# akhilmurthy/spacedrive

Measured on AMD Instinct MI355X. Metric: cas_id files/sec + BLAKE3 GB/s hashed (node) at 1/2/4/8 MI355X, higher is better.
Workload: dtype u32

## Files before the change

### spacedrive_amd/csrc/b3_batch.h

```cpp
#pragma once
#include <hip/hip_runtime.h>
#include <stddef.h>
#include <stdint.h>

namespace sdcas {

constexpr uint32_t kTile = 1024;
constexpr uint32_t kWG = 512;
constexpr uint32_t kSmallTile = 128;
constexpr uint64_t kSmallSlots = 1ull << 14;
constexpr int kSmallVariant = 84;
constexpr uint32_t kSortTotalsWords = 256;
constexpr uint32_t kSortPerWG = 4096;
inline size_t sort_key_words(size_t max_msgs) { return kSortTotalsWords + 256 * (max_msgs / kSortPerWG + 1); }

struct BatchWorkspace {
  uint64_t* S = nullptr;
  uint32_t* tile_first = nullptr;
  uint64_t* total = nullptr;
  uint32_t* nodes = nullptr;
  void* scan_tmp = nullptr;
  size_t scan_tmp_bytes = 0;
  uint32_t cap_msgs = 0;
  uint64_t cap_chunks = 0;
  uint64_t cap_slots = 0;
  int variant = -1;
  uint64_t small_slots = kSmallSlots;
  int small_variant = kSmallVariant;
  uint64_t cap_small_tiles = 0;
  int sort = 1;
  uint32_t* perm = nullptr;
  uint64_t* soffs = nullptr;
  uint64_t* slens = nullptr;
  uint32_t* sort_keys = nullptr;
};

size_t batch_scan_temp_bytes(uint32_t max_msgs);
int leaf_variant();
int leaf_variant_count();
bool leaf_variant_available(int v);
bool leaf_variant_forced();
bool piece_variant_available(int v);

constexpr uint32_t kSortMinMsgs = 128;
struct BatchPlan {
  const uint64_t* S = nullptr;
  const uint32_t* tile_first = nullptr;
  uint64_t* total = nullptr;
  uint32_t tile = 0;
  bool crossing = true;
};
uint64_t batch_plan_host(const uint64_t* lens, uint32_t n, uint32_t tile, uint64_t cap_slots, uint64_t* S,
                         uint32_t* tile_first, uint64_t* total, bool* crossing);

hipError_t batch_hash(const BatchWorkspace& ws, const uint8_t* blob, const uint64_t* offs, const uint64_t* lens,
                      uint32_t n, uint8_t* out32, uint64_t* out_keys, hipStream_t st, uint64_t max_chunks = 0,
                      hipEvent_t ev0 = nullptr, hipEvent_t ev1 = nullptr, const BatchPlan* plan = nullptr);

hipError_t plan_slots(const uint64_t* lens, uint32_t n, void* tmp, size_t tmp_bytes, uint64_t cap_slots, uint64_t* S,
                      uint32_t* tile_first, uint64_t* total, hipStream_t st);
hipError_t finish_crossing(uint64_t tiles, const uint64_t* lens, uint32_t n, const uint64_t* S,
                           const uint32_t* tile_first, const uint64_t* total, uint64_t cap_slots,
                           const uint32_t* nodes, uint8_t* out32, uint64_t* out_keys, hipStream_t st);

constexpr uint64_t kWholeMax = 102400;
constexpr uint64_t kGatherStride = 57360;
constexpr uint32_t kIdentifyMaxSampled = 4096;
struct IdentifyScratch {
  uint8_t* p = nullptr;
  size_t bytes = 0;
};
size_t identify_scratch_bytes(uint32_t n, uint32_t sampled_cap);
hipError_t identify_hash(const BatchWorkspace& ws, const IdentifyScratch& sc, const uint8_t* blob,
                         const uint64_t* offs, const uint64_t* lens, uint32_t n, uint32_t sampled_cap,
                         uint64_t* out_keys, uint8_t* out32, uint8_t* out_has_key, hipStream_t st);

struct PieceDesc {
  uint64_t off;
  uint64_t j0;
  uint64_t node_base;
  uint32_t len;
  uint32_t pad;
};
struct SegDesc {
  uint64_t off;
  uint64_t j0;
  uint64_t node_base;
  uint64_t len;
  uint64_t piece_first;
};
struct FileDesc {
  uint64_t C;
  uint64_t node_base;
  uint64_t out_index;
};
inline uint64_t bigfile_node_count(uint64_t C) {
  return C / kTile + (uint64_t)__builtin_popcountll(C % kTile);
// ... 11 lines not shown
```

### spacedrive_amd/csrc/b3_batch.hip

```cpp
#include <hip/hip_runtime.h>

#include <atomic>
#ifdef SDCAS_ABLATIONS
#include <hipcub/hipcub.hpp>
#endif
#include <stdint.h>
#include <cstdio>
#include <cstring>

#include "b3_device.h"
#include "b3_batch.h"
#include "b3_tree.h"

namespace sdcas {

using namespace b3d;

constexpr int kMaxStack = 64;
constexpr int kMaxStackBig = 64;


template <uint32_t TILE = kTile>
__global__ void k_tile_first(const uint64_t* __restrict__ lens, const uint64_t* __restrict__ S, uint32_t n,
                             uint64_t cap_chunks, uint32_t* __restrict__ tile_first, uint64_t* __restrict__ total) {
// ... 372 lines not shown
    static_assert(L == 8 || L == 9 || L == 4 || L == 59 || L == 69 || L == 79 || L == 89, "ablation block loops need -DSDCAS_ABLATIONS");
#endif
  }
}

template <int PF>
__device__ __forceinline__ const uint8_t* leaf_ptr(const uint8_t* blob, const uint8_t* p) {
#ifdef SDCAS_ABLATIONS
  return leaf_ptr_ablation<PF>(blob, p);
#else
  (void)blob;
  return p;
#endif
}

__device__ __forceinline__ uint32_t leaf_bin(uint64_t len, uint64_t j) {
  const uint64_t rest = len - j * CHUNK_LEN;
  const uint32_t clen = len == 0 ? 0u : (uint32_t)min<uint64_t>(CHUNK_LEN, rest);
  const uint32_t nb = clen == 0 ? 1u : (clen + BLOCK_LEN - 1) / BLOCK_LEN;
  return 16u - nb;
}


template <int WG, uint32_t NB = 17, uint32_t TL = kTile>
__device__ __forceinline__ void leaf_order(uint32_t tid, const uint32_t (&bin)[TL / WG], uint16_t* __restrict__ order,
                                           uint16_t* __restrict__ gcnt) {
  constexpr uint32_t kGroups = TL / 64;
  const uint32_t lane = tid & 63;
  uint32_t rk[TL / WG];
#pragma unroll
  for (uint32_t r = 0; r < TL / WG; ++r) {
    const uint32_t g = (tid + r * WG) >> 6;
    uint32_t mine = 0, cnt_l = 0;
#pragma unroll 1
    for (uint32_t b = 0; b < NB; ++b) {
      const uint64_t m = __ballot(bin[r] == b);
      if (bin[r] == b) mine = __builtin_amdgcn_mbcnt_hi((uint32_t)(m >> 32), __builtin_amdgcn_mbcnt_lo((uint32_t)m, 0u));
      if (lane == b) cnt_l = (uint32_t)__popcll(m);
    }
    rk[r] = mine;
    if (lane < NB) gcnt[lane * kGroups + g] = (uint16_t)cnt_l;
  }
  __syncthreads();
  if (tid < 64) {
    constexpr uint32_t kPer = (NB * kGroups + 63) / 64;
    uint32_t v[kPer], sum = 0;
#pragma unroll
    for (uint32_t q = 0; q < kPer; ++q) {
      const uint32_t e = tid * kPer + q;
      v[q] = e < NB * kGroups ? gcnt[e] : 0u;
      sum += v[q];
    }
    uint32_t inc = sum;
#pragma unroll
    for (uint32_t d = 1; d < 64; d <<= 1) {
      const uint32_t t = __shfl_up(inc, d);
      if (lane >= d) inc += t;
    }
    uint32_t acc = inc - sum;
#pragma unroll
    for (uint32_t q = 0; q < kPer; ++q) {
      const uint32_t e = tid * kPer + q;
      if (e < NB * kGroups) gcnt[e] = (uint16_t)acc;
      acc += v[q];
    }
  }
  __syncthreads();
#pragma unroll
  for (uint32_t r = 0; r < TL / WG; ++r) {
    const uint32_t s = tid + r * WG;
    order[gcnt[bin[r] * kGroups + (s >> 6)] + rk[r]] = (uint16_t)s;
  }
  __syncthreads();
}

template <int WG, int PF, int TR = 1, int ORD = 0, int DYN = 0, int CA = 0, int MINW = 0, uint32_t TL = kTile,
          int QD = 0, int XT = 0>
__global__ void __launch_bounds__(WG, MINW ? MINW : (ORD ? 6 : 1)) k_leaf_tree(const uint8_t* __restrict__ blob, const uint64_t* __restrict__ offs,
                                                   const uint64_t* __restrict__ lens, uint32_t n,
                                                   const uint64_t* __restrict__ S,
                                                   const uint32_t* __restrict__ tile_first,
                                                   const uint64_t* __restrict__ total_p, uint64_t cap_chunks,
                                                   uint32_t* __restrict__ nodes, uint8_t* __restrict__ out32,
                                                   uint64_t* __restrict__ out_keys, const uint32_t* __restrict__ perm) {
  __shared__ uint32_t cvs[TL][8];
  __shared__ uint64_t sS[TL + 1];
  __shared__ uint16_t smsg[TL];
  __shared__ uint32_t task[kTaskCap<TL>];
  __shared__ uint32_t ntask[12];
  __shared__ uint16_t order[ORD ? TL : 1];
  __shared__ uint32_t sexp[(XT & 2) ? TL / 32 : 1];
  __shared__ uint64_t next_tile;
  __shared__ uint32_t qbuf[QD == 3 ? 16 * (WG / 4) : 1];

  if constexpr (((XT >> 3) & 7) != 0) asm volatile(".rept %c0\n s_nop 0\n .endr" ::"i"((XT >> 3) & 7));
  const uint64_t total = *total_p;
  if (total > cap_chunks) return;
  const uint64_t ntiles = (total + TL - 1) / TL;
  const uint32_t tid = threadIdx.x;
  static_assert(!QD || (ORD == 0 && CA == 0 && WG % 4 == 0), "quad slots: no leaf order, no cached chunk");
  constexpr uint32_t SW = QD ? WG / 4 : WG;
  const uint32_t sid = QD ? tid >> 2 : tid;
  const bool lead = !QD || (tid & 3u) == 0;
  const uint32_t qslot = 16 * sid;
  uint32_t wi[QD == 3 ? 28 : 1];
  if constexpr (QD == 3) {
    const uint32_t q = tid & 3u;
    const bool q1 = q & 1u, q2 = q & 2u;
#pragma unroll
    for (int k = 0; k < 28; ++k)
      wi[k] = qslot + qsel(q1, q2, kQuadWord.w[0][k], kQuadWord.w[1][k], kQuadWord.w[2][k], kQuadWord.w[3][k]);
  }
  unsigned long long* tile_ctr = reinterpret_cast<unsigned long long*>(const_cast<uint64_t*>(total_p) + 2);
  for (uint64_t tile = blockIdx.x; tile < ntiles;) {
    const uint64_t tbase = tile * TL;
    const uint32_t m0 = tile_first[tile];
    const uint32_t m1 = (tile + 1 < ntiles) ? tile_first[tile + 1] : n - 1;
    const uint32_t cnt = m1 - m0 + 1;
    for (uint32_t i = tid; i < cnt; i += WG) sS[i] = S[m0 + i];
    if (tid < 12) ntask[tid] = 0;
    if constexpr ((XT & 2) != 0)
      for (uint32_t i = tid; i < TL / 32; i += WG) sexp[i] = 0;
    if (DYN == 1 && tid == 0) next_tile = gridDim.x + atomicAdd(tile_ctr, 1ull);
    __syncthreads();

    constexpr uint32_t R = TL / SW;
    const uint8_t* c_p[R];
    uint64_t c_j[R];
    uint32_t c_clen[R], c_m[R];
    bool c_ok[R], c_root[R];
#pragma unroll
    for (uint32_t r = 0; r < R; ++r) c_ok[r] = false;
    constexpr uint32_t kPhase1Unroll = CA ? R : 1;
#pragma unroll kPhase1Unroll
    for (uint32_t s = sid; s < TL; s += SW) {
      const uint64_t g = tbase + s;
      uint32_t K = 0;
      if (g >= total) {
        smsg[s] = kNoMsg;
      } else {
        uint32_t lo = 0, hi = cnt - 1;
        while (lo < hi) {
          const uint32_t mid = (lo + hi + 1) >> 1;
          if (sS[mid] <= g) lo = mid;
          else hi = mid - 1;
        }
        smsg[s] = (uint16_t)lo;
        if (TR || CA) {
          const uint64_t j = g - sS[lo];
          const uint64_t len = lens[m0 + lo];
          const uint64_t C = chunk_count(len);
          if (CA && (CA == 1 || s == tid)) {
            const uint32_t r = (s - tid) / WG;
            c_ok[r] = true;
            c_m[r] = m0 + lo;
            c_j[r] = j;
            c_clen[r] = len == 0 ? 0u : (uint32_t)min<uint64_t>(CHUNK_LEN, len - j * CHUNK_LEN);
            c_root[r] = C == 1;
            c_p[r] = blob + offs[m0 + lo] + j * CHUNK_LEN;
          }
          if (TR && C != 1 && lead) {
            K = node_level_t<TL>(j, C, s);
            if constexpr ((XT & 4) == 0)
              for (uint32_t k = 1; k <= K; ++k)
                task[task_base<TL>(k) + atomicAdd(&ntask[k], 1u)] = enc_task(s, s + (1u << (k - 1)), 0, false);
            if constexpr ((XT & 2) != 0) {
              const uint64_t S0 = g - j;
              if ((S0 < tbase || S0 + C > tbase + TL) && !parent_in_tile_t<TL>(j, C, s, K))
                atomicOr(&sexp[s >> 5], 1u << (s & 31));
            }
          }
        }
      }
      if constexpr ((XT & 4) != 0) {
        for (uint32_t k = 1;; ++k) {
          const bool want = K >= k;
          const uint64_t bal = __ballot(want);
          if (!bal) break;
          const uint32_t first = (uint32_t)__ffsll((long long)bal) - 1;
          uint32_t base = 0;
          if (__lane_id() == first) base = atomicAdd(&ntask[k], (uint32_t)__popcll(bal));
          base = __shfl(base, (int)first);
          const uint32_t below =
              __builtin_amdgcn_mbcnt_hi((uint32_t)(bal >> 32), __builtin_amdgcn_mbcnt_lo((uint32_t)bal, 0u));
          if (want) task[task_base<TL>(k) + base + below] = enc_task(s, s + (1u << (k - 1)), 0, false);
        }
      }
    }
#pragma unroll 1
    for (uint32_t i = sid; TR && lead && i < cnt; i += SW) {
      const uint64_t S0 = sS[i];
      if (S0 < tbase) continue;
      const uint64_t C = chunk_count(lens[m0 + i]);
      if (C == 1 || S0 + C > tbase + TL) continue;
      const uint32_t s0 = (uint32_t)(S0 - tbase), c = (uint32_t)C;
      if (!(c & (c - 1))) {
        const uint32_t k = 31 - __clz(c);
// ... 218 lines not shown
template <uint32_t TILE, bool QUAD = false, class At>
__device__ __forceinline__ void merge_nodes_flat(const uint32_t* __restrict__ nodes, uint64_t s0, uint64_t C, At at,
                                                 uint32_t (&cv)[8]) {
  int depth = 0, keep = 0;
  uint64_t j = 0;
  uint32_t k = 0;
  bool have = false, done = false;
  uint32_t v[8];
  for (;;) {
    int op = 0;
    while (!done) {
      if (!have) {
        const uint64_t g = s0 + j;
        k = node_level_t<TILE>(j, C, (uint32_t)(g % TILE));
        const uint4* p = reinterpret_cast<const uint4*>(nodes + 8ull * g);
        const uint4 a = p[0], b = p[1];
        v[0] = a.x; v[1] = a.y; v[2] = a.z; v[3] = a.w;
        v[4] = b.x; v[5] = b.y; v[6] = b.z; v[7] = b.w;
        keep = __popcll(j);
        have = true;
      }
      if (depth > keep) {
        op = 1;
        break;
      }
      if (j + (1ull << k) < C) {
        uint32_t* pp = at(depth);
#pragma unroll
        for (int i = 0; i < 8; ++i) pp[i] = v[i];
        ++depth;
        j += 1ull << k;
        have = false;
        continue;
      }
      if (depth == 0) {
#pragma unroll
        for (int i = 0; i < 8; ++i) cv[i] = v[i];
        done = true;
        break;
      }
      op = 2;
      break;
    }
    if (__builtin_amdgcn_ballot_w64(op != 0) == 0) return;
    if (op) {
      uint32_t l[8], r[8], o[8];
      const uint32_t* pl = at(op == 1 ? depth - 2 : depth - 1);
      const uint32_t* pr = at(depth - 1);
#pragma unroll
      for (int i = 0; i < 8; ++i) {
        l[i] = pl[i];
        r[i] = op == 1 ? pr[i] : v[i];
      }
      if constexpr (QUAD) parent_quad(l, r, op == 2 && depth == 1, o);
      else parent(l, r, op == 2 && depth == 1, o);
      if (op == 1) {
        uint32_t* po = at(depth - 2);
#pragma unroll
        for (int i = 0; i < 8; ++i) po[i] = o[i];
      } else {
#pragma unroll
        for (int i = 0; i < 8; ++i) v[i] = o[i];
      }
      --depth;
    }
  }
}

template <uint32_t TILE>
__device__ __noinline__ void merge_nodes_deep(const uint32_t* __restrict__ nodes, uint64_t s0, uint64_t C,
                                              uint32_t (&cv)[8]) {
  uint32_t stack[kMaxStack][8];
  merge_nodes<TILE>(nodes, s0, C, [&](int d) { return &stack[d][0]; }, cv);
}

constexpr int kFinishWG = 64, kFinishDepth = 24;
template <uint32_t TILE>
__global__ void __launch_bounds__(kFinishWG) k_finish_t(const uint64_t* __restrict__ lens, uint32_t n,
                                                       const uint64_t* __restrict__ S,
                                                       const uint32_t* __restrict__ tile_first,
                                                       const uint64_t* __restrict__ total_p, uint64_t cap_slots,
                                                       const uint32_t* __restrict__ nodes,
                                                       const uint32_t* __restrict__ perm, uint8_t* __restrict__ out32,
                                                       uint64_t* __restrict__ out_keys) {
  constexpr uint32_t kFinishRow = kFinishDepth * 8 + 1;
  __shared__ uint32_t lstack[kFinishWG][kFinishRow];
  const uint64_t t = (uint64_t)blockIdx.x * blockDim.x + threadIdx.x;
  const uint64_t total = *total_p;
  if (total > cap_slots || t == 0 || t * TILE >= total) return;
  const uint32_t m = tile_first[t];
  const uint64_t s0 = S[m];
  if (s0 >= t * TILE || s0 / TILE != t - 1) return;
  const uint64_t C = chunk_count(lens[m]);
  if (s0 + C <= t * TILE) return;
  uint32_t cv[8];
  if (C < (1ull << (kFinishDepth - 2)))
    merge_nodes_flat<TILE>(nodes, s0, C, [&](int d) { return &lstack[threadIdx.x][8 * d]; }, cv);
  else
    merge_nodes_deep<TILE>(nodes, s0, C, cv);
  store_digest(perm ? perm[m] : m, cv, out32, out_keys);
}

constexpr int kFinishQWG = 64, kFinishQPerWG = kFinishQWG / 4;
template <uint32_t TILE>
__global__ void __launch_bounds__(kFinishQWG) k_finish_q(const uint64_t* __restrict__ lens, uint32_t n,
                                                        const uint64_t* __restrict__ S,
                                                        const uint32_t* __restrict__ tile_first,
                                                        const uint64_t* __restrict__ total_p, uint64_t cap_slots,
                                                        const uint32_t* __restrict__ nodes,
                                                        const uint32_t* __restrict__ perm, uint8_t* __restrict__ out32,
                                                        uint64_t* __restrict__ out_keys) {
  constexpr uint32_t kFinishRow = kFinishDepth * 8 + 1;
  __shared__ uint32_t lstack[kFinishQPerWG][kFinishRow];
  const uint32_t b = threadIdx.x >> 2;
  const uint64_t t = (uint64_t)blockIdx.x * kFinishQPerWG + b;
  const uint64_t total = *total_p;
  if (total > cap_slots || t == 0 || t * TILE >= total) return;
  const uint32_t m = tile_first[t];
  const uint64_t s0 = S[m];
  if (s0 >= t * TILE || s0 / TILE != t - 1) return;
  const uint64_t C = chunk_count(lens[m]);
  if (s0 + C <= t * TILE) return;
  uint32_t cv[8];
  if (C < (1ull << (kFinishDepth - 2)))
    merge_nodes_flat<TILE, true>(nodes, s0, C, [&](int d) { return &lstack[b][8 * d]; }, cv);
  else
    merge_nodes_deep<TILE>(nodes, s0, C, cv);
  if ((threadIdx.x & 3) == 0) store_digest(perm ? perm[m] : m, cv, out32, out_keys);
}

static bool finish_by_quad() {
  const char* v = getenv("SDCAS_FINISH");
  return !(v && strcmp(v, "lane") == 0);
}

template <uint32_t TILE>
static void launch_finish(uint64_t tiles, hipStream_t st, const uint64_t* lens, uint32_t n, const uint64_t* S,
                          const uint32_t* tile_first, const uint64_t* total, uint64_t cap_slots, const uint32_t* nodes,
                          const uint32_t* perm, uint8_t* out32, uint64_t* out_keys) {
  if (finish_by_quad())
    hipLaunchKernelGGL(k_finish_q<TILE>, dim3((uint32_t)((tiles + kFinishQPerWG - 1) / kFinishQPerWG)),
                       dim3(kFinishQWG), 0, st, lens, n, S, tile_first, total, cap_slots, nodes, perm, out32,
                       out_keys);
  else
    hipLaunchKernelGGL(k_finish_t<TILE>, dim3((uint32_t)((tiles + kFinishWG - 1) / kFinishWG)), dim3(kFinishWG), 0,
                       st, lens, n, S, tile_first, total, cap_slots, nodes, perm, out32, out_keys);
}

#ifdef SDCAS_ABLATIONS
#include "b3_ablate_kernels.inc"
#endif

constexpr uint32_t kShapeBins = 256;
constexpr uint32_t kScatterPerWG = 4096;
constexpr uint32_t kScatterR = kScatterPerWG / 256;
constexpr uint32_t kShapeManyChunks = 15 << 4;
static_assert(kSortTotalsWords == kShapeBins && kSortPerWG == kScatterPerWG, "ws.sort_keys layout");

__device__ __forceinline__ uint32_t shape_key(uint64_t L) {
  const uint64_t C = chunk_count(L);
  const uint64_t last = L - (C - 1) * CHUNK_LEN;
  const uint32_t blocks = last == 0 ? 1u : (uint32_t)((last + BLOCK_LEN - 1) / BLOCK_LEN);
  return ((uint32_t)min<uint64_t>(C, 15) << 4) | (blocks - 1);
}

__global__ void __launch_bounds__(256) k_shape_hist(const uint64_t* __restrict__ lens, uint32_t n,
                                                    uint32_t* __restrict__ wcnt) {
  __shared__ uint32_t h[kShapeBins];
  const uint32_t t = threadIdx.x;
  h[t] = 0;
  __syncthreads();
  const uint64_t lo = (uint64_t)blockIdx.x * kScatterPerWG;
  uint64_t L[kScatterR];
#pragma unroll
  for (uint32_t r = 0; r < kScatterR; ++r) {
    const uint64_t i = lo + r * 256 + t;
    L[r] = i < n ? lens[i] : 0;
  }
#pragma unroll
  for (uint32_t r = 0; r < kScatterR; ++r)
    if (lo + r * 256 + t < n) atomicAdd(&h[shape_key(L[r])], 1u);
  __syncthreads();
  wcnt[(uint64_t)t * gridDim.x + blockIdx.x] = h[t];
}

__global__ void __launch_bounds__(256) k_shape_bins(uint32_t* __restrict__ wcnt, uint32_t nwg,
                                                    uint32_t* __restrict__ totals) {
  __shared__ uint32_t ws[4];
  __shared__ uint32_t carry;
  const uint32_t t = threadIdx.x, lane = t & 63, wave = t >> 6;
  uint32_t* col = wcnt + (uint64_t)blockIdx.x * nwg;
  if (t == 0) carry = 0;
  __syncthreads();
  for (uint32_t base = 0; base < nwg; base += 256) {
    const uint32_t i = base + t;
    const uint32_t v = i < nwg ? col[i] : 0u;
    uint32_t inc = v;
#pragma unroll
    for (uint32_t d = 1; d < 64; d <<= 1) {
      const uint32_t x = __shfl_up(inc, d);
      if (lane >= d) inc += x;
    }
    if (lane == 63) ws[wave] = inc;
    __syncthreads();
    uint32_t before = carry;
    for (uint32_t w = 0; w < wave; ++w) before += ws[w];
    if (i < nwg) col[i] = before + inc - v;
    __syncthreads();
    if (t == 255) carry = before + inc;
    __syncthreads();
  }
  if (t == 0) totals[blockIdx.x] = carry;
}

__global__ void __launch_bounds__(256) k_shape_scatter(const uint64_t* __restrict__ offs,
                                                       const uint64_t* __restrict__ lens, uint32_t n,
                                                       const uint32_t* __restrict__ totals,
                                                       const uint32_t* __restrict__ wstart,
                                                       uint32_t* __restrict__ perm, uint64_t* __restrict__ soffs,
                                                       uint64_t* __restrict__ slens) {
  __shared__ uint32_t gstart[kShapeBins], lstart[kShapeBins], h[kShapeBins];
  __shared__ uint16_t order[kScatterPerWG];
  __shared__ uint8_t keyof[kScatterPerWG];
  __shared__ uint32_t few_chunks;
  const uint32_t t = threadIdx.x;
  const uint32_t bin_count = totals[t];
  gstart[t] = bin_count;
  h[t] = 0;
  __syncthreads();
  for (uint32_t d = 1; d < kShapeBins; d <<= 1) {
    const uint32_t v = t >= d ? gstart[t - d] : 0u;
    __syncthreads();
    gstart[t] += v;
    __syncthreads();
  }
  if (t == kShapeManyChunks - 1) few_chunks = gstart[t];
  const uint32_t excl = gstart[t] - bin_count;
  __syncthreads();
  gstart[t] = excl;
  const uint32_t lo = blockIdx.x * kScatterPerWG, hi = min(n, lo + kScatterPerWG), m = hi - lo;
  if ((uint64_t)(n - few_chunks) * 10 > (uint64_t)n * 6) {
    uint64_t o[kScatterR], l[kScatterR];
#pragma unroll
    for (uint32_t r = 0; r < kScatterR; ++r) {
      const uint32_t k = t + r * 256;
      o[r] = k < m ? offs[lo + k] : 0;
      l[r] = k < m ? lens[lo + k] : 0;
    }
#pragma unroll
    for (uint32_t r = 0; r < kScatterR; ++r) {
      const uint32_t k = t + r * 256;
      if (k >= m) continue;
      perm[lo + k] = lo + k;
      soffs[lo + k] = o[r];
      slens[lo + k] = l[r];
    }
    return;
  }
  {
    uint64_t l[kScatterR];
#pragma unroll
    for (uint32_t r = 0; r < kScatterR; ++r) {
      const uint32_t k = t + r * 256;
      l[r] = k < m ? lens[lo + k] : 0;
    }
#pragma unroll
    for (uint32_t r = 0; r < kScatterR; ++r) {
      const uint32_t k = t + r * 256;
      if (k >= m) continue;
      const uint32_t key = shape_key(l[r]);
      keyof[k] = (uint8_t)key;
      atomicAdd(&h[key], 1u);
    }
  }
  __syncthreads();
  const uint32_t cnt = h[t];
  gstart[t] += wstart[(uint64_t)t * gridDim.x + blockIdx.x];
  lstart[t] = cnt;
  __syncthreads();
  for (uint32_t d = 1; d < kShapeBins; d <<= 1) {
    const uint32_t v = t >= d ? lstart[t - d] : 0u;
    __syncthreads();
    lstart[t] += v;
    __syncthreads();
  }
  lstart[t] -= cnt;
  h[t] = 0;
  __syncthreads();
  for (uint32_t k = t; k < m; k += 256) {
    const uint32_t key = keyof[k];
    order[lstart[key] + atomicAdd(&h[key], 1u)] = (uint16_t)k;
  }
  __syncthreads();
  uint32_t kk[kScatterR];
  uint64_t o[kScatterR], l[kScatterR];
#pragma unroll
  for (uint32_t r = 0; r < kScatterR; ++r) {
    const uint32_t p = t + r * 256;
    kk[r] = p < m ? order[p] : 0u;
    o[r] = p < m ? offs[lo + kk[r]] : 0;
    l[r] = p < m ? lens[lo + kk[r]] : 0;
  }
#pragma unroll
  for (uint32_t r = 0; r < kScatterR; ++r) {
    const uint32_t p = t + r * 256;
    if (p >= m) continue;
    const uint32_t key = keyof[kk[r]];
    const uint32_t pos = gstart[key] + (p - lstart[key]);
    perm[pos] = lo + kk[r];
    soffs[pos] = o[r];
    slens[pos] = l[r];
  }
}



template <int PF, int DIRECT, int ROT, int TOP, int DEFER>
__device__ __forceinline__ void piece_pass(const uint8_t* __restrict__ blob, const PieceDesc* __restrict__ pieces,
                                           uint32_t npieces, uint32_t* __restrict__ file_nodes,
                                           uint32_t* __restrict__ l4) {
  __shared__ uint32_t cvs[kTile][8];
  __shared__ uint16_t task[kTile / 2];
  __shared__ uint32_t ntask[16];
  const uint32_t tid = threadIdx.x;
  for (uint32_t pi = blockIdx.x; pi < npieces; pi += gridDim.x) {
    const PieceDesc pd = pieces[pi];
    const uint32_t nchunks = (pd.len + CHUNK_LEN - 1) / CHUNK_LEN;
    if (tid < 16) ntask[tid] = 0;
    const uint32_t rot = ROT ? (uint32_t)((pi * 7u * 64u) % nchunks) & ~63u : 0u;
#pragma unroll 1
    for (uint32_t s0 = tid; s0 < nchunks; s0 += kWG) {
      uint32_t s = s0 + rot;
      if (ROT && s >= nchunks) s -= nchunks;
      const uint32_t clen = min(CHUNK_LEN, pd.len - s * CHUNK_LEN);
      uint32_t cv[8];
      leaf_hash<PF>(blob + pd.off + (uint64_t)s * CHUNK_LEN, clen, pd.j0 + s, false, cv);
#pragma unroll
      for (int i = 0; i < 8; ++i) cvs[s][i] = cv[i];
    }
    __syncthreads();
    const bool defer = DEFER && nchunks == kTile;
    const uint32_t top = defer ? kPieceDeferLevel : TOP;
    for (uint32_t k = 1; (1u << k) <= kTile && k <= top; ++k) {
      const uint32_t w = 1u << k;
      uint32_t T;
      if (DIRECT) {
        T = nchunks >> k;
        if (T == 0) break;
      } else {
        for (uint32_t s = tid; s < nchunks; s += kWG)
          if (!(s & (w - 1)) && s + w <= nchunks) task[atomicAdd(&ntask[k], 1u)] = (uint16_t)s;
        __syncthreads();
        T = ntask[k];
        if (T == 0) break;
      }
#pragma unroll 1
      for (uint32_t t = tid; t < T; t += kWG) {
        const uint32_t s = DIRECT ? t << k : task[t];
        uint32_t l[8], r[8], o[8];
#pragma unroll
        for (int i = 0; i < 8; ++i) {
          l[i] = cvs[s][i];
          r[i] = cvs[s + (w >> 1)][i];
        }
        parent<kGA<PF>>(l, r, false, o);
#pragma unroll
        for (int i = 0; i < 8; ++i) cvs[s][i] = o[i];
      }
      __syncthreads();
    }
    if (defer) {
      for (uint32_t t = tid; t < kTile >> kPieceDeferLevel; t += kWG) {
        const uint32_t s = t << kPieceDeferLevel;
        uint4* o = reinterpret_cast<uint4*>(l4 + 8ull * ((uint64_t)pi * (kTile >> kPieceDeferLevel) + t));
        o[0] = make_uint4(cvs[s][0], cvs[s][1], cvs[s][2], cvs[s][3]);
        o[1] = make_uint4(cvs[s][4], cvs[s][5], cvs[s][6], cvs[s][7]);
      }
      __syncthreads();
      continue;
    }
    for (uint32_t s = tid; s < nchunks; s += kWG) {
      const uint32_t rest = nchunks - s;
      const uint32_t k = 31 - __clz(rest);
      if ((s & ((1u << k) - 1)) || (s != (nchunks & ~((2u << k) - 1)))) continue;
      const uint64_t idx = pd.node_base + (nchunks == kTile ? pd.j0 / kTile : pd.j0 / kTile + __popc(nchunks >> (k + 1)));
      uint4* o = reinterpret_cast<uint4*>(file_nodes + 8ull * idx);
      o[0] = make_uint4(cvs[s][0], cvs[s][1], cvs[s][2], cvs[s][3]);
      o[1] = make_uint4(cvs[s][4], cvs[s][5], cvs[s][6], cvs[s][7]);
    }
    __syncthreads();
  }
}

template <int PF, int MINW, int DIRECT = 0, int ROT = 0, int TOP = 10>
// ... 428 lines not shown
#undef ABL
#undef ABLQ
#undef RET
constexpr int kNumLeafVariants = sizeof(kLeafVariants) / sizeof(kLeafVariants[0]);
constexpr int kDefaultLeafVariant = 67;

int leaf_variant_count() { return kNumLeafVariants; }
bool leaf_variant_forced() {
  static const bool f = [] {
    const char* e = getenv("SDCAS_LEAF_VARIANT");
    return e && leaf_variant_available(atoi(e));
  }();
  return f;
}
bool leaf_variant_available(int v) { return v >= 0 && v < kNumLeafVariants && kLeafVariants[v].fn != nullptr; }

int leaf_variant() {
  static const int v = [] {
    const char* e = getenv("SDCAS_LEAF_VARIANT");
    const int x = e ? atoi(e) : kDefaultLeafVariant;
    return leaf_variant_available(x) ? x : kDefaultLeafVariant;
  }();
  return v;
}

int batch_grid(int device, int variant) {
  static std::atomic<int> cached[64][kNumLeafVariants];
  const bool cacheable = device >= 0 && device < 64 && variant >= 0 && variant < kNumLeafVariants;
  if (cacheable && cached[device][variant].load(std::memory_order_relaxed))
    return cached[device][variant].load(std::memory_order_relaxed);
  int cus = 256, per = 1;
  (void)hipDeviceGetAttribute(&cus, hipDeviceAttributeMultiprocessorCount, device);
  (void)hipOccupancyMaxActiveBlocksPerMultiprocessor(&per, kLeafVariants[variant].fn, kLeafVariants[variant].wg, 0);
  if (per < 1) per = 1;
  if (getenv("SDCAS_DEBUG_GRID")) fprintf(stderr, "leaf variant %d: %d workgroups/CU\n", variant, per);
  int g = cus * per;
  if (cacheable) cached[device][variant].store(g, std::memory_order_relaxed);
  return g;
}

uint64_t batch_plan_host(const uint64_t* lens, uint32_t n, uint32_t tile, uint64_t cap_slots, uint64_t* S,
                         uint32_t* tile_first, uint64_t* total, bool* crossing) {
  uint64_t s = 0, tiles = 0;
  bool cross = false;
  for (uint32_t m = 0; m < n; ++m) {
    const uint64_t C = chunk_count(lens[m]);
    S[m] = s;
    for (uint64_t t = (s + tile - 1) / tile; t * tile < s + C && t * tile < cap_slots; ++t) tile_first[t] = m;
    cross |= s / tile != (s + C - 1) / tile;
    s += C;
  }
  tiles = (s + tile - 1) / tile;
  total[0] = s;
  total[1] = total[2] = total[3] = 0;
  *crossing = cross;
  return tiles;
}

hipError_t plan_slots(const uint64_t* lens, uint32_t n, void* tmp, size_t tmp_bytes, uint64_t cap_slots, uint64_t* S,
                      uint32_t* tile_first, uint64_t* total, hipStream_t st) {
  const uint32_t nb = (n + kPlanPer - 1) / kPlanPer;
  if ((size_t)(nb + 1) * sizeof(uint64_t) > tmp_bytes) return hipErrorInvalidValue;
  uint64_t* bsum = static_cast<uint64_t*>(tmp);
  hipLaunchKernelGGL(k_plan_sums, dim3(nb), dim3(kPlanWG), 0, st, lens, n, bsum);
  hipLaunchKernelGGL(k_plan_scan, dim3(1), dim3(1024), 0, st, bsum, nb, total);
  hipLaunchKernelGGL(k_plan_write<kTile>, dim3(nb), dim3(kPlanWG), 0, st, lens, n, bsum, cap_slots, S, tile_first);
  return hipGetLastError();
}

hipError_t finish_crossing(uint64_t tiles, const uint64_t* lens, uint32_t n, const uint64_t* S,
                           const uint32_t* tile_first, const uint64_t* total, uint64_t cap_slots,
                           const uint32_t* nodes, uint8_t* out32, uint64_t* out_keys, hipStream_t st) {
  launch_finish<kTile>(tiles, st, lens, n, S, tile_first, total, cap_slots, nodes, nullptr, out32, out_keys);
  return hipGetLastError();
}

hipError_t batch_hash(const BatchWorkspace& ws, const uint8_t* blob, const uint64_t* offs, const uint64_t* lens,
                      uint32_t n, uint8_t* out32, uint64_t* out_keys, hipStream_t st, uint64_t max_chunks,
                      hipEvent_t ev0, hipEvent_t ev1, const BatchPlan* plan) {
  if (n == 0) return hipSuccess;
  if (n > ws.cap_msgs) return hipErrorInvalidValue;
  [[maybe_unused]] hipError_t e;
  const uint32_t* perm = nullptr;
  if (ws.sort && n >= kSortMinMsgs && ws.perm) {
    const uint32_t nwg = (n + kScatterPerWG - 1) / kScatterPerWG;
    uint32_t* totals = ws.sort_keys;
    uint32_t* wcnt = ws.sort_keys + kSortTotalsWords;
    hipLaunchKernelGGL(k_shape_hist, dim3(nwg), dim3(256), 0, st, lens, n, wcnt);
    hipLaunchKernelGGL(k_shape_bins, dim3(kShapeBins), dim3(256), 0, st, wcnt, nwg, totals);
    hipLaunchKernelGGL(k_shape_scatter, dim3(nwg), dim3(256), 0, st, offs, lens, n, totals, wcnt, ws.perm, ws.soffs,
                       ws.slens);
    offs = ws.soffs;
    lens = ws.slens;
    perm = ws.perm;
  }
  const bool forced = leaf_variant_available(ws.variant) || leaf_variant_forced();
  int v = leaf_variant_available(ws.variant) ? ws.variant : leaf_variant();
  bool quad = false;
#ifdef SDCAS_ABLATIONS
  quad = kLeafVariants[v].quad && (perm || n == 1);
  if (kLeafVariants[v].quad && !quad) v = kDefaultLeafVariant;
#endif
  const uint64_t slots =
      max_chunks ? std::min<uint64_t>(ws.cap_slots, max_chunks + (quad ? 3ull * n + 8 : 0)) : ws.cap_slots;
  if (!forced && !quad && slots <= ws.small_slots && slots / kSmallTile + 2 <= ws.cap_small_tiles)
    v = leaf_variant_available(ws.small_variant) && kLeafVariants[ws.small_variant].tile == kSmallTile ? ws.small_variant
                                                                                                        : kSmallVariant;
  if (kLeafVariants[v].tile == kSmallTile && slots / kSmallTile + 2 > ws.cap_small_tiles) v = kDefaultLeafVariant;
  const uint32_t tile = kLeafVariants[v].tile;
  const bool planned = plan && !perm && !quad && plan->tile == tile;
  uint64_t* const S = planned ? const_cast<uint64_t*>(plan->S) : ws.S;
  uint32_t* const tile_first = planned ? const_cast<uint32_t*>(plan->tile_first) : ws.tile_first;
  uint64_t* const total = planned ? plan->total : ws.total;
  size_t tmp = ws.scan_tmp_bytes;
  if (planned) {
  } else if (quad) {
#ifdef SDCAS_ABLATIONS
    QuadIt qit(hipcub::CountingInputIterator<uint32_t>(0), QuadSlotsOp{lens, n});
    if ((e = hipcub::DeviceScan::ExclusiveSum(ws.scan_tmp, tmp, qit, ws.S, (int)n, st))) return e;
    hipLaunchKernelGGL(k_tile_first_q, dim3((n + 255) / 256), dim3(256), 0, st, lens, ws.S, n, ws.cap_slots,
                       ws.tile_first, ws.total);
#endif
  } else {
    const uint32_t nb = (n + kPlanPer - 1) / kPlanPer;
    if ((size_t)(nb + 1) * sizeof(uint64_t) > tmp) return hipErrorInvalidValue;
    uint64_t* bsum = static_cast<uint64_t*>(ws.scan_tmp);
    hipLaunchKernelGGL(k_plan_sums, dim3(nb), dim3(kPlanWG), 0, st, lens, n, bsum);
    hipLaunchKernelGGL(k_plan_scan, dim3(1), dim3(1024), 0, st, bsum, nb, ws.total);
    if (tile == kSmallTile)
      hipLaunchKernelGGL(k_plan_write<kSmallTile>, dim3(nb), dim3(kPlanWG), 0, st, lens, n, bsum, ws.cap_slots, ws.S,
                         ws.tile_first);
    else
      hipLaunchKernelGGL(k_plan_write<kTile>, dim3(nb), dim3(kPlanWG), 0, st, lens, n, bsum, ws.cap_slots, ws.S,
                         ws.tile_first);
  }
  if (ev0) (void)hipEventRecord(ev0, st);
  {
    int dev = 0;
    (void)hipGetDevice(&dev);
    const int grid = kLeafVariants[v].one_tile ? (int)std::min<uint64_t>(slots / tile + 1, 0x7FFFFFFF)
                                               : batch_grid(dev, v);
    void* args[] = {(void*)&blob,     (void*)&offs,       (void*)&lens,     (void*)&n,
                    (void*)&S,        (void*)&tile_first, (void*)&total,    (void*)&ws.cap_slots,
                    (void*)&ws.nodes, (void*)&out32,      (void*)&out_keys, (void*)&perm};
    hipError_t le = hipLaunchKernel(kLeafVariants[v].fn, dim3(grid), dim3(kLeafVariants[v].wg), args, 0, st);
    if (le != hipSuccess) return le;
  }
  if (ev1) (void)hipEventRecord(ev1, st);
  if (quad) {
#ifdef SDCAS_ABLATIONS
    const uint64_t tiles = slots / kQTile + 1;
    hipLaunchKernelGGL(k_finish_t<kQTile>, dim3((uint32_t)((tiles + kFinishWG - 1) / kFinishWG)), dim3(kFinishWG), 0,
                       st, lens, n, ws.S, ws.tile_first, ws.total, ws.cap_slots, ws.nodes, perm, out32, out_keys);
#endif
  } else if (planned && !plan->crossing) {
  } else if (tile == kSmallTile) {
    launch_finish<kSmallTile>(slots / kSmallTile + 1, st, lens, n, S, tile_first, total, ws.cap_slots, ws.nodes, perm,
                              out32, out_keys);
  } else {
    launch_finish<kTile>(slots / kTile + 1, st, lens, n, S, tile_first, total, ws.cap_slots, ws.nodes, perm, out32,
                         out_keys);
  }
  return hipGetLastError();
}

constexpr int kDefaultPieceVariant = 19;

bool piece_variant_available(int v) {
  if (v == 17 || v == 19) return true;
#ifdef SDCAS_ABLATIONS
  if (v >= 0 && v <= 20) return true;
#endif
  return false;
}

int piece_variant() {
  static const int v = [] {
    const char* e = getenv("SDCAS_PIECE_VARIANT");
    const int x = e ? atoi(e) : kDefaultPieceVariant;
    return piece_variant_available(x) ? x : kDefaultPieceVariant;
  }();
  return v;
}

#ifdef SDCAS_ABLATIONS
static int piece_grid(const void* fn) {
  int dev = 0, cus = 0, per = 0;
  (void)hipGetDevice(&dev);
  (void)hipDeviceGetAttribute(&cus, hipDeviceAttributeMultiprocessorCount, dev);
  (void)hipOccupancyMaxActiveBlocksPerMultiprocessor(&per, fn, kWG, 0);
  return (cus > 0 ? cus : 256) * (per > 0 ? per : 1);
}

template <int MINW, int PRE>
static hipError_t launch_piece_dyn(const uint8_t* blob, const PieceDesc* pieces, uint32_t npieces,
                                   uint32_t* file_nodes, uint32_t* ctr, hipStream_t st) {
  static int grid = 0;
  if (!grid) grid = piece_grid((const void*)k_piece_dyn<MINW, PRE>);
  hipError_t e = hipMemsetAsync(ctr, 0, sizeof(uint32_t), st);
  if (e) return e;
  hipLaunchKernelGGL((k_piece_dyn<MINW, PRE>), dim3(std::min<uint32_t>(npieces, (uint32_t)grid)), dim3(kWG), 0, st,
                     blob, pieces, npieces, file_nodes, ctr);
  return hipGetLastError();
}

static hipError_t piece_hash_ablation(int v, const uint8_t* blob, const PieceDesc* pieces, uint32_t npieces,
                                      uint32_t* file_nodes, uint32_t* ctr, uint32_t* l4, hipStream_t st) {
  if (v == 20) {
    if (!l4) return hipErrorInvalidValue;
    hipLaunchKernelGGL((k_piece_l4<259, 8>), dim3(npieces), dim3(kWG), 0, st, blob, pieces, npieces, file_nodes, l4);
    hipLaunchKernelGGL((k_piece_top<259>), dim3((npieces + kTopPieces - 1) / kTopPieces), dim3(kWG), 0, st, pieces,
                       npieces, l4, file_nodes);
    return hipGetLastError();
  }
  if (v == 11) return launch_piece_dyn<6, 0>(blob, pieces, npieces, file_nodes, ctr, st);
  if (v == 12) return launch_piece_dyn<6, 1>(blob, pieces, npieces, file_nodes, ctr, st);
  if (v == 13) return launch_piece_dyn<8, 0>(blob, pieces, npieces, file_nodes, ctr, st);
  if (v == 16)
    hipLaunchKernelGGL((k_piece_tree<208, 6, 1, 0, 4>), dim3(npieces), dim3(kWG), 0, st, blob, pieces, npieces,
                       file_nodes);
  else if (v == 14)
    hipLaunchKernelGGL((k_piece_tree<108, 6, 1>), dim3(npieces), dim3(kWG), 0, st, blob, pieces, npieces, file_nodes);
  else if (v == 18)
    hipLaunchKernelGGL((k_piece_tree<259, 6, 1, 0, 4>), dim3(npieces), dim3(kWG), 0, st, blob, pieces, npieces,
                       file_nodes);
  else if (v == 15)
    hipLaunchKernelGGL((k_piece_tree<208, 6, 1>), dim3(npieces), dim3(kWG), 0, st, blob, pieces, npieces, file_nodes);
  if (v >= 14) return hipGetLastError();
  if (v == 0) hipLaunchKernelGGL((k_piece_tree<0, 1>), dim3(npieces), dim3(kWG), 0, st, blob, pieces, npieces, file_nodes);
  else if (v == 1)
    hipLaunchKernelGGL((k_piece_tree<1, 8>), dim3(npieces), dim3(kWG), 0, st, blob, pieces, npieces, file_nodes);
  else if (v == 2)
    hipLaunchKernelGGL((k_piece_tree<1, 8, 1>), dim3(npieces), dim3(kWG), 0, st, blob, pieces, npieces, file_nodes);
  else if (v == 3)
    hipLaunchKernelGGL((k_piece_tree<1, 6, 1>), dim3(npieces), dim3(kWG), 0, st, blob, pieces, npieces, file_nodes);
  else if (v == 5)
    hipLaunchKernelGGL((k_piece_tree<4, 8, 1>), dim3(npieces), dim3(kWG), 0, st, blob, pieces, npieces, file_nodes);
  else if (v == 6)
    hipLaunchKernelGGL((k_piece_tree<8, 6, 1>), dim3(npieces), dim3(kWG), 0, st, blob, pieces, npieces, file_nodes);
  else if (v == 7)
    hipLaunchKernelGGL((k_piece_tree<2, 6, 1>), dim3(npieces), dim3(kWG), 0, st, blob, pieces, npieces, file_nodes);
  else if (v == 8)
    hipLaunchKernelGGL((k_piece_tree<4, 6, 1, 1>), dim3(npieces), dim3(kWG), 0, st, blob, pieces, npieces, file_nodes);
  else if (v == 9)
// ... 70 lines not shown
```

Before: 62.45 million.

## Fuse slot planning into shape-sort scatter and add heavy-first tile order

The shape histogram and bin-scan kernels now also accumulate per-bin chunk sums. This lets the scatter kernel compute slot offsets S, tile_first and total directly, so the separate plan_sums/plan_scan/plan_write pass is skipped on the sorted path. When input order is kept, the scatter no longer copies offs/lens/perm. Instead the leaf and finish kernels read the original arrays via a flag in total[3]. A heavy-first reversed tile start order is also added for the dynamic default variant. This trades fewer launches and less copy traffic for a more complex scatter kernel with extra shared memory and scans.

Result: no change. 62.47 million (median of 2 runs) (+0.0%).

```diff
diff --git a/spacedrive_amd/csrc/b3_batch.h b/spacedrive_amd/csrc/b3_batch.h
--- a/spacedrive_amd/csrc/b3_batch.h
+++ b/spacedrive_amd/csrc/b3_batch.h
@@ -12,7 +12,11 @@
 constexpr int kSmallVariant = 84;
 constexpr uint32_t kSortTotalsWords = 256;
 constexpr uint32_t kSortPerWG = 4096;
-inline size_t sort_key_words(size_t max_msgs) { return kSortTotalsWords + 256 * (max_msgs / kSortPerWG + 1); }
+constexpr uint32_t kSortSumCols = 17;
+inline size_t sort_key_words(size_t max_msgs) {
+  const size_t wgs = max_msgs / kSortPerWG + 1;
+  return kSortTotalsWords + 256 * wgs + 2 * (kSortSumCols * wgs + kSortSumCols);
+}
 
 struct BatchWorkspace {
   uint64_t* S = nullptr;
diff --git a/spacedrive_amd/csrc/b3_batch.hip b/spacedrive_amd/csrc/b3_batch.hip
--- a/spacedrive_amd/csrc/b3_batch.hip
+++ b/spacedrive_amd/csrc/b3_batch.hip
@@ -478,7 +478,9 @@
                                                    const uint32_t* __restrict__ tile_first,
                                                    const uint64_t* __restrict__ total_p, uint64_t cap_chunks,
                                                    uint32_t* __restrict__ nodes, uint8_t* __restrict__ out32,
-                                                   uint64_t* __restrict__ out_keys, const uint32_t* __restrict__ perm) {
+                                                   uint64_t* __restrict__ out_keys, const uint32_t* __restrict__ perm,
+                                                   uint32_t heavy_first, const uint64_t* __restrict__ offs_c,
+                                                   const uint64_t* __restrict__ lens_c) {
   __shared__ uint32_t cvs[TL][8];
   __shared__ uint64_t sS[TL + 1];
   __shared__ uint16_t smsg[TL];
@@ -508,7 +510,15 @@
       wi[k] = qslot + qsel(q1, q2, kQuadWord.w[0][k], kQuadWord.w[1][k], kQuadWord.w[2][k], kQuadWord.w[3][k]);
   }
   unsigned long long* tile_ctr = reinterpret_cast<unsigned long long*>(const_cast<uint64_t*>(total_p) + 2);
-  for (uint64_t tile = blockIdx.x; tile < ntiles;) {
+  const bool kept = lens_c != nullptr && total_p[3] != 0;
+  if (kept) {
+    offs = offs_c;
+    lens = lens_c;
+    perm = nullptr;
+  }
+  uint64_t tile = blockIdx.x;
+  if (DYN == 2 && heavy_first && !kept && tile < ntiles) tile = ntiles - 1 - tile;
+  for (; tile < ntiles;) {
     const uint64_t tbase = tile * TL;
     const uint32_t m0 = tile_first[tile];
     const uint32_t m1 = (tile + 1 < ntiles) ? tile_first[tile + 1] : n - 1;
@@ -893,12 +903,17 @@
                                                        const uint64_t* __restrict__ total_p, uint64_t cap_slots,
                                                        const uint32_t* __restrict__ nodes,
                                                        const uint32_t* __restrict__ perm, uint8_t* __restrict__ out32,
-                                                       uint64_t* __restrict__ out_keys) {
+                                                       uint64_t* __restrict__ out_keys,
+                                                       const uint64_t* __restrict__ lens_c) {
   constexpr uint32_t kFinishRow = kFinishDepth * 8 + 1;
   __shared__ uint32_t lstack[kFinishWG][kFinishRow];
   const uint64_t t = (uint64_t)blockIdx.x * blockDim.x + threadIdx.x;
   const uint64_t total = *total_p;
   if (total > cap_slots || t == 0 || t * TILE >= total) return;
+  if (lens_c && total_p[3]) {
+    lens = lens_c;
+    perm = nullptr;
+  }
   const uint32_t m = tile_first[t];
   const uint64_t s0 = S[m];
   if (s0 >= t * TILE || s0 / TILE != t - 1) return;
@@ -920,13 +935,18 @@
                                                         const uint64_t* __restrict__ total_p, uint64_t cap_slots,
                                                         const uint32_t* __restrict__ nodes,
                                                         const uint32_t* __restrict__ perm, uint8_t* __restrict__ out32,
-                                                        uint64_t* __restrict__ out_keys) {
+                                                        uint64_t* __restrict__ out_keys,
+                                                        const uint64_t* __restrict__ lens_c) {
   constexpr uint32_t kFinishRow = kFinishDepth * 8 + 1;
   __shared__ uint32_t lstack[kFinishQPerWG][kFinishRow];
   const uint32_t b = threadIdx.x >> 2;
   const uint64_t t = (uint64_t)blockIdx.x * kFinishQPerWG + b;
   const uint64_t total = *total_p;
   if (total > cap_slots || t == 0 || t * TILE >= total) return;
+  if (lens_c && total_p[3]) {
+    lens = lens_c;
+    perm = nullptr;
+  }
   const uint32_t m = tile_first[t];
   const uint64_t s0 = S[m];
   if (s0 >= t * TILE || s0 / TILE != t - 1) return;
@@ -945,17 +965,26 @@
   return !(v && strcmp(v, "lane") == 0);
 }
 
+static bool tile_order_heavy_first() {
+  static const bool on = [] {
+    const char* v = getenv("SDCAS_TILE_ORDER");
+    return !(v && strcmp(v, "asc") == 0);
+  }();
+  return on;
+}
+
 template <uint32_t TILE>
 static void launch_finish(uint64_t tiles, hipStream_t st, const uint64_t* lens, uint32_t n, const uint64_t* S,
                           const uint32_t* tile_first, const uint64_t* total, uint64_t cap_slots, const uint32_t* nodes,
-                          const uint32_t* perm, uint8_t* out32, uint64_t* out_keys) {
+                          const uint32_t* perm, uint8_t* out32, uint64_t* out_keys,
+                          const uint64_t* lens_c = nullptr) {
   if (finish_by_quad())
     hipLaunchKernelGGL(k_finish_q<TILE>, dim3((uint32_t)((tiles + kFinishQPerWG - 1) / kFinishQPerWG)),
                        dim3(kFinishQWG), 0, st, lens, n, S, tile_first, total, cap_slots, nodes, perm, out32,
-                       out_keys);
+                       out_keys, lens_c);
   else
     hipLaunchKernelGGL(k_finish_t<TILE>, dim3((uint32_t)((tiles + kFinishWG - 1) / kFinishWG)), dim3(kFinishWG), 0,
-                       st, lens, n, S, tile_first, total, cap_slots, nodes, perm, out32, out_keys);
+                       st, lens, n, S, tile_first, total, cap_slots, nodes, perm, out32, out_keys, lens_c);
 }
 
 #ifdef SDCAS_ABLATIONS
@@ -967,6 +996,9 @@
 constexpr uint32_t kScatterR = kScatterPerWG / 256;
 constexpr uint32_t kShapeManyChunks = 15 << 4;
 static_assert(kSortTotalsWords == kShapeBins && kSortPerWG == kScatterPerWG, "ws.sort_keys layout");
+constexpr uint32_t kShapeManyBins = kShapeBins - kShapeManyChunks;
+constexpr uint32_t kShapeSumCols = kShapeManyBins + 1;
+static_assert(kSortSumCols == kShapeSumCols, "ws.sort_keys layout");
 
 __device__ __forceinline__ uint32_t shape_key(uint64_t L) {
   const uint64_t C = chunk_count(L);
@@ -976,10 +1008,12 @@
 }
 
 __global__ void __launch_bounds__(256) k_shape_hist(const uint64_t* __restrict__ lens, uint32_t n,
-                                                    uint32_t* __restrict__ wcnt) {
+                                                    uint32_t* __restrict__ wcnt, uint64_t* __restrict__ wsum) {
   __shared__ uint32_t h[kShapeBins];
+  __shared__ unsigned long long cs[kShapeSumCols];
   const uint32_t t = threadIdx.x;
   h[t] = 0;
+  if (t < kShapeSumCols) cs[t] = 0;
   __syncthreads();
   const uint64_t lo = (uint64_t)blockIdx.x * kScatterPerWG;
   uint64_t L[kScatterR];
@@ -988,18 +1022,52 @@
     const uint64_t i = lo + r * 256 + t;
     L[r] = i < n ? lens[i] : 0;
   }
-#pragma unroll
-  for (uint32_t r = 0; r < kScatterR; ++r)
-    if (lo + r * 256 + t < n) atomicAdd(&h[shape_key(L[r])], 1u);
+  uint64_t all = 0;
+#pragma unroll
+  for (uint32_t r = 0; r < kScatterR; ++r) {
+    if (lo + r * 256 + t >= n) continue;
+    const uint32_t key = shape_key(L[r]);
+    const uint64_t C = chunk_count(L[r]);
+    atomicAdd(&h[key], 1u);
+    if (key >= kShapeManyChunks) atomicAdd(&cs[key - kShapeManyChunks], (unsigned long long)C);
+    all += C;
+  }
+#pragma unroll
+  for (uint32_t d = 32; d; d >>= 1) all += __shfl_xor(all, d);
+  if ((t & 63) == 0) atomicAdd(&cs[kShapeManyBins], (unsigned long long)all);
   __syncthreads();
   wcnt[(uint64_t)t * gridDim.x + blockIdx.x] = h[t];
+  if (t < kShapeSumCols) wsum[(uint64_t)t * gridDim.x + blockIdx.x] = cs[t];
 }
 
 __global__ void __launch_bounds__(256) k_shape_bins(uint32_t* __restrict__ wcnt, uint32_t nwg,
-                                                    uint32_t* __restrict__ totals) {
+                                                    uint32_t* __restrict__ totals, uint64_t* __restrict__ wsum,
+                                                    uint64_t* __restrict__ stotals) {
   __shared__ uint32_t ws[4];
   __shared__ uint32_t carry;
   const uint32_t t = threadIdx.x, lane = t & 63, wave = t >> 6;
+  if (blockIdx.x >= kShapeBins) {
+    __shared__ uint64_t ws8[4];
+    __shared__ uint64_t carry8;
+    uint64_t* col8 = wsum + (uint64_t)(blockIdx.x - kShapeBins) * nwg;
+    if (t == 0) carry8 = 0;
+    __syncthreads();
+    for (uint32_t base = 0; base < nwg; base += 256) {
+      const uint32_t i = base + t;
+      const uint64_t v = i < nwg ? col8[i] : 0;
+      const uint64_t inc = wave_incl_scan(v, lane);
+      if (lane == 63) ws8[wave] = inc;
+      __syncthreads();
+      uint64_t before = carry8;
+      for (uint32_t w = 0; w < wave; ++w) before += ws8[w];
+      if (i < nwg) col8[i] = before + inc - v;
+      __syncthreads();
+      if (t == 255) carry8 = before + inc;
+      __syncthreads();
+    }
+    if (t == 0) stotals[blockIdx.x - kShapeBins] = carry8;
+    return;
+  }
   uint32_t* col = wcnt + (uint64_t)blockIdx.x * nwg;
   if (t == 0) carry = 0;
   __syncthreads();
@@ -1024,47 +1092,119 @@
   if (t == 0) totals[blockIdx.x] = carry;
 }
 
-__global__ void __launch_bounds__(256) k_shape_scatter(const uint64_t* __restrict__ offs,
+
+__device__ __forceinline__ uint64_t scatter_scan_round(uint64_t c, uint32_t r, uint64_t& run, uint64_t (&ws)[2][4]) {
+  const uint32_t lane = threadIdx.x & 63, wave = threadIdx.x >> 6;
+  const uint64_t inc = wave_incl_scan(c, lane);
+  if (lane == 63) ws[r & 1][wave] = inc;
+  __syncthreads();
+  uint64_t before = run;
+#pragma unroll
+  for (uint32_t w = 0; w < 4; ++w) {
+    const uint64_t x = ws[r & 1][w];
+    if (w < wave) before += x;
+    run += x;
+  }
+  return before + inc - c;
+}
+
+__device__ __forceinline__ void mark_tiles(uint64_t s0, uint64_t C, uint32_t m, uint32_t tile_shift,
+                                           uint64_t cap_slots, uint32_t* __restrict__ tile_first) {
+  const uint64_t tm = (1ull << tile_shift) - 1;
+  for (uint64_t t = (s0 + tm) >> tile_shift; (t << tile_shift) < s0 + C && (t << tile_shift) < cap_slots; ++t)
+    tile_first[t] = m;
+}
+
+__global__ void __launch_bounds__(256, 4) k_shape_scatter(const uint64_t* __restrict__ offs,
                                                        const uint64_t* __restrict__ lens, uint32_t n,
                                                        const uint32_t* __restrict__ totals,
                                                        const uint32_t* __restrict__ wstart,
-                                                       uint32_t* __restrict__ perm, uint64_t* __restrict__ soffs,
-                                                       uint64_t* __restrict__ slens) {
+                                                       const uint64_t* __restrict__ wsum,
+                                                       const uint64_t* __restrict__ stotals, uint32_t tile_shift,
+                                                       uint64_t cap_slots, uint32_t copy_kept,
+                                                       uint32_t* __restrict__ perm,
+                                                       uint64_t* __restrict__ soffs, uint64_t* __restrict__ slens,
+                                                       uint64_t* __restrict__ S, uint32_t* __restrict__ tile_first,
+                                                       uint64_t* __restrict__ total) {
   __shared__ uint32_t gstart[kShapeBins], lstart[kShapeBins], h[kShapeBins];
+  __shared__ uint64_t sstart[kShapeBins];
+  __shared__ uint64_t own15[kShapeManyBins];
+  __shared__ uint64_t scan_ws[2][4];
   __shared__ uint16_t order[kScatterPerWG];
   __shared__ uint8_t keyof[kScatterPerWG];
   __shared__ uint32_t few_chunks;
   const uint32_t t = threadIdx.x;
   const uint32_t bin_count = totals[t];
+  const uint64_t bin_slots =
+      t < kShapeManyChunks ? (uint64_t)bin_count * (t >> 4) : stotals[t - kShapeManyChunks];
+  const uint64_t wbase = wsum[(uint64_t)kShapeManyBins * gridDim.x + blockIdx.x];
+  const uint64_t run_slots =
+      t < kShapeManyChunks ? 0 : wsum[(uint64_t)(t - kShapeManyChunks) * gridDim.x + blockIdx.x];
+  if (t >= kShapeManyChunks) {
+    const uint64_t next = blockIdx.x + 1 < gridDim.x
+                              ? wsum[(uint64_t)(t - kShapeManyChunks) * gridDim.x + blockIdx.x + 1]
+                              : bin_slots;
+    own15[t - kShapeManyChunks] = next - run_slots;
+  }
   gstart[t] = bin_count;
+  sstart[t] = bin_slots;
   h[t] = 0;
   __syncthreads();
   for (uint32_t d = 1; d < kShapeBins; d <<= 1) {
     const uint32_t v = t >= d ? gstart[t - d] : 0u;
+    const uint64_t sv = t >= d ? sstart[t - d] : 0;
     __syncthreads();
     gstart[t] += v;
+    sstart[t] += sv;
     __syncthreads();
   }
   if (t == kShapeManyChunks - 1) few_chunks = gstart[t];
   const uint32_t excl = gstart[t] - bin_count;
+  const uint64_t sexcl = sstart[t] - bin_slots;
+  const uint64_t all_slots = sstart[kShapeBins - 1];
   __syncthreads();
   gstart[t] = excl;
+  sstart[t] = sexcl;
   const uint32_t lo = blockIdx.x * kScatterPerWG, hi = min(n, lo + kScatterPerWG), m = hi - lo;
-  if ((uint64_t)(n - few_chunks) * 10 > (uint64_t)n * 6) {
-    uint64_t o[kScatterR], l[kScatterR];
+  const bool keep_order = (uint64_t)(n - few_chunks) * 10 > (uint64_t)n * 6;
+  if (blockIdx.x == 0 && t == 0) {
+    total[0] = all_slots;
+    total[2] = 0;
+    total[3] = keep_order;
+  }
+  if (keep_order) {
+    uint64_t l[kScatterR];
 #pragma unroll
     for (uint32_t r = 0; r < kScatterR; ++r) {
       const uint32_t k = t + r * 256;
-      o[r] = k < m ? offs[lo + k] : 0;
       l[r] = k < m ? lens[lo + k] : 0;
     }
+    if (copy_kept) {
+      uint64_t o[kScatterR];
+#pragma unroll
+      for (uint32_t r = 0; r < kScatterR; ++r) {
+        const uint32_t k = t + r * 256;
+        o[r] = k < m ? offs[lo + k] : 0;
+      }
+#pragma unroll
+      for (uint32_t r = 0; r < kScatterR; ++r) {
+        const uint32_t k = t + r * 256;
+        if (k >= m) continue;
+        perm[lo + k] = lo + k;
+        soffs[lo + k] = o[r];
+        slens[lo + k] = l[r];
+      }
+    }
+    uint64_t run = wbase;
 #pragma unroll
     for (uint32_t r = 0; r < kScatterR; ++r) {
+      if (r * 256 >= m) continue;
       const uint32_t k = t + r * 256;
+      const uint64_t C = k < m ? chunk_count(l[r]) : 0;
+      const uint64_t s0 = scatter_scan_round(C, r, run, scan_ws);
       if (k >= m) continue;
-      perm[lo + k] = lo + k;
-      soffs[lo + k] = o[r];
-      slens[lo + k] = l[r];
+      S[lo + k] = s0;
+      mark_tiles(s0, C, lo + k, tile_shift, cap_slots, tile_first);
     }
     return;
   }
@@ -1086,7 +1226,15 @@
   }
   __syncthreads();
   const uint32_t cnt = h[t];
-  gstart[t] += wstart[(uint64_t)t * gridDim.x + blockIdx.x];
+  const uint32_t before = wstart[(uint64_t)t * gridDim.x + blockIdx.x];
+  gstart[t] += before;
+  if (t < kShapeManyChunks) {
+    sstart[t] += (uint64_t)before * (t >> 4);
+  } else {
+    uint64_t earlier = 0;
+    for (uint32_t k = 0; k < t - kShapeManyChunks; ++k) earlier += own15[k];
+    sstart[t] += run_slots - earlier;
+  }
   lstart[t] = cnt;
   __syncthreads();
   for (uint32_t d = 1; d < kShapeBins; d <<= 1) {
@@ -1117,10 +1265,31 @@
     const uint32_t p = t + r * 256;
     if (p >= m) continue;
     const uint32_t key = keyof[kk[r]];
-    const uint32_t pos = gstart[key] + (p - lstart[key]);
+    const uint32_t rank = p - lstart[key], pos = gstart[key] + rank;
     perm[pos] = lo + kk[r];
     soffs[pos] = o[r];
     slens[pos] = l[r];
+    if (key < kShapeManyChunks) {
+      const uint64_t s0 = sstart[key] + (uint64_t)rank * (key >> 4);
+      S[pos] = s0;
+      mark_tiles(s0, key >> 4, pos, tile_shift, cap_slots, tile_first);
+    }
+  }
+  const uint32_t many0 = lstart[kShapeManyChunks];
+  uint64_t run = 0;
+#pragma unroll
+  for (uint32_t r = 0; r < kScatterR; ++r) {
+    if ((r + 1) * 256 <= many0 || r * 256 >= m) continue;
+    const uint32_t p = t + r * 256;
+    const bool many = p < m && p >= many0;
+    const uint64_t C = many ? chunk_count(l[r]) : 0;
+    const uint64_t before = scatter_scan_round(C, r, run, scan_ws);
+    if (!many) continue;
+    const uint32_t key = keyof[kk[r]];
+    const uint32_t pos = gstart[key] + (p - lstart[key]);
+    const uint64_t s0 = sstart[key] + before;
+    S[pos] = s0;
+    mark_tiles(s0, C, pos, tile_shift, cap_slots, tile_first);
   }
 }
 
@@ -1715,23 +1884,13 @@
   if (n > ws.cap_msgs) return hipErrorInvalidValue;
   [[maybe_unused]] hipError_t e;
   const uint32_t* perm = nullptr;
-  if (ws.sort && n >= kSortMinMsgs && ws.perm) {
-    const uint32_t nwg = (n + kScatterPerWG - 1) / kScatterPerWG;
-    uint32_t* totals = ws.sort_keys;
-    uint32_t* wcnt = ws.sort_keys + kSortTotalsWords;
-    hipLaunchKernelGGL(k_shape_hist, dim3(nwg), dim3(256), 0, st, lens, n, wcnt);
-    hipLaunchKernelGGL(k_shape_bins, dim3(kShapeBins), dim3(256), 0, st, wcnt, nwg, totals);
-    hipLaunchKernelGGL(k_shape_scatter, dim3(nwg), dim3(256), 0, st, offs, lens, n, totals, wcnt, ws.perm, ws.soffs,
-                       ws.slens);
-    offs = ws.soffs;
-    lens = ws.slens;
-    perm = ws.perm;
-  }
+  const uint64_t *offs_c = nullptr, *lens_c = nullptr;
+  const bool sorted = ws.sort && n >= kSortMinMsgs && ws.perm;
   const bool forced = leaf_variant_available(ws.variant) || leaf_variant_forced();
   int v = leaf_variant_available(ws.variant) ? ws.variant : leaf_variant();
   bool quad = false;
 #ifdef SDCAS_ABLATIONS
-  quad = kLeafVariants[v].quad && (perm || n == 1);
+  quad = kLeafVariants[v].quad && (sorted || n == 1);
   if (kLeafVariants[v].quad && !quad) v = kDefaultLeafVariant;
 #endif
   const uint64_t slots =
@@ -1741,6 +1900,31 @@
                                                                                                         : kSmallVariant;
   if (kLeafVariants[v].tile == kSmallTile && slots / kSmallTile + 2 > ws.cap_small_tiles) v = kDefaultLeafVariant;
   const uint32_t tile = kLeafVariants[v].tile;
+  if (sorted) {
+    const uint32_t nwg = (n + kScatterPerWG - 1) / kScatterPerWG;
+    uint32_t* totals = ws.sort_keys;
+    uint32_t* wcnt = ws.sort_keys + kSortTotalsWords;
+    uint64_t* wsum = reinterpret_cast<uint64_t*>(wcnt + (size_t)kShapeBins * nwg);
+    uint64_t* stotals = wsum + (size_t)kShapeSumCols * nwg;
+    const uint32_t tile_shift = tile == kSmallTile ? 7u : 10u;
+    static_assert(kSmallTile == 1u << 7 && kTile == 1u << 10, "tile_shift");
+    hipLaunchKernelGGL(k_shape_hist, dim3(nwg), dim3(256), 0, st, lens, n, wcnt, wsum);
+    hipLaunchKernelGGL(k_shape_bins, dim3(kShapeBins + kShapeSumCols), dim3(256), 0, st, wcnt, nwg, totals, wsum,
+                       stotals);
+#ifdef SDCAS_ABLATIONS
+    const uint32_t copy_kept = 1;
+#else
+    const uint32_t copy_kept = 0;
+#endif
+    hipLaunchKernelGGL(k_shape_scatter, dim3(nwg), dim3(256), 0, st, offs, lens, n, totals, wcnt, wsum, stotals,
+                       tile_shift, ws.cap_slots, copy_kept, ws.perm, ws.soffs, ws.slens, ws.S, ws.tile_first,
+                       ws.total);
+    offs_c = offs;
+    lens_c = lens;
+    offs = ws.soffs;
+    lens = ws.slens;
+    perm = ws.perm;
+  }
   const bool planned = plan && !perm && !quad && plan->tile == tile;
   uint64_t* const S = planned ? const_cast<uint64_t*>(plan->S) : ws.S;
   uint32_t* const tile_first = planned ? const_cast<uint32_t*>(plan->tile_first) : ws.tile_first;
@@ -1754,6 +1938,7 @@
     hipLaunchKernelGGL(k_tile_first_q, dim3((n + 255) / 256), dim3(256), 0, st, lens, ws.S, n, ws.cap_slots,
                        ws.tile_first, ws.total);
 #endif
+  } else if (sorted) {
   } else {
     const uint32_t nb = (n + kPlanPer - 1) / kPlanPer;
     if ((size_t)(nb + 1) * sizeof(uint64_t) > tmp) return hipErrorInvalidValue;
@@ -1773,9 +1958,11 @@
     (void)hipGetDevice(&dev);
     const int grid = kLeafVariants[v].one_tile ? (int)std::min<uint64_t>(slots / tile + 1, 0x7FFFFFFF)
                                                : batch_grid(dev, v);
+    uint32_t heavy_first = sorted && !quad && v == kDefaultLeafVariant && tile_order_heavy_first();
     void* args[] = {(void*)&blob,     (void*)&offs,       (void*)&lens,     (void*)&n,
                     (void*)&S,        (void*)&tile_first, (void*)&total,    (void*)&ws.cap_slots,
-                    (void*)&ws.nodes, (void*)&out32,      (void*)&out_keys, (void*)&perm};
+                    (void*)&ws.nodes, (void*)&out32,      (void*)&out_keys, (void*)&perm,
+                    (void*)&heavy_first, (void*)&offs_c,    (void*)&lens_c};
     hipError_t le = hipLaunchKernel(kLeafVariants[v].fn, dim3(grid), dim3(kLeafVariants[v].wg), args, 0, st);
     if (le != hipSuccess) return le;
   }
@@ -1784,15 +1971,16 @@
 #ifdef SDCAS_ABLATIONS
     const uint64_t tiles = slots / kQTile + 1;
     hipLaunchKernelGGL(k_finish_t<kQTile>, dim3((uint32_t)((tiles + kFinishWG - 1) / kFinishWG)), dim3(kFinishWG), 0,
-                       st, lens, n, ws.S, ws.tile_first, ws.total, ws.cap_slots, ws.nodes, perm, out32, out_keys);
+                       st, lens, n, ws.S, ws.tile_first, ws.total, ws.cap_slots, ws.nodes, perm, out32, out_keys,
+                       (const uint64_t*)nullptr);
 #endif
   } else if (planned && !plan->crossing) {
   } else if (tile == kSmallTile) {
     launch_finish<kSmallTile>(slots / kSmallTile + 1, st, lens, n, S, tile_first, total, ws.cap_slots, ws.nodes, perm,
-                              out32, out_keys);
+                              out32, out_keys, lens_c);
   } else {
     launch_finish<kTile>(slots / kTile + 1, st, lens, n, S, tile_first, total, ws.cap_slots, ws.nodes, perm, out32,
-                         out_keys);
+                         out_keys, lens_c);
   }
   return hipGetLastError();
 }
```
